# videosegmentation/video_segment

Hardware: AMD Instinct MI355X
Metric: over-segmented frames/sec at 1080p (higher is better)
Workload: dtype f32

## Files before the change

### video_segment_amd/csrc/dense_graph.cpp

```cpp
#include "dense_graph.h"
#include "scan_device.h"

#include <algorithm>
#include <chrono>
#include <cmath>
#include <cstring>
#include <atomic>
#include <functional>
#include <thread>
#include <unordered_set>

namespace vsg {

namespace {
template <class T>
DevBuf<T>& Grow(DevBuf<T>& b, size_t n) {
  if (b.size() < n) b.alloc(n + n / 2 + 1024);
  return b;
}
double NowMs() {
  using clk = std::chrono::steady_clock;
  return std::chrono::duration<double, std::milli>(clk::now().time_since_epoch()).count();
}
template <class T>
// ... 577 lines not shown
  const int window_bushy = getenv("VSG_WINDOW_BUSHY") ? atoi(getenv("VSG_WINDOW_BUSHY")) : 64;
  const bool adapt_windows = !getenv("VSG_ADAPT_WINDOWS") || atoi(getenv("VSG_ADAPT_WINDOWS")) != 0;
  const int window_min_edges =
      getenv("VSG_WINDOW_MIN") ? atoi(getenv("VSG_WINDOW_MIN")) : (int)std::min<size_t>(2 * wh_, 1u << 30);
  const int window_min_replayed =
      getenv("VSG_WINDOW_MIN_REPLAYED") ? atoi(getenv("VSG_WINDOW_MIN_REPLAYED"))
                                        : (getenv("VSG_WINDOW_MIN") ? 0 : (int)std::min<size_t>(wh_ / 2, 1u << 30));
  S.bucket_prefix = bucket_prefix_dev_.get();
  S.bucket_prefix_host = bucket_prefix.data();
  {
    list_off_host_.assign((size_t)L * (kNumBuckets + 2), 0);
    for (int l = 0; l < L; ++l) {
      int32_t* off = list_off_host_.data() + (size_t)l * (kNumBuckets + 2);
      int acc_l = 0;
      for (int b = 0; b <= kNumBuckets; ++b) {
        off[b] = acc_l;
        const int32_t* row = bucket_base_host_.data() + (size_t)b * (L + 1);
        acc_l += row[l + 1] - row[l];
      }
      off[kNumBuckets + 1] = acc_l;
    }
    const size_t cap = (size_t)3 * 65536;
    if (seg_table_dev_.size() < cap) seg_table_dev_.alloc(cap);
    S.bucket_base_host = getenv("VSG_FILTER_SEGS") && atoi(getenv("VSG_FILTER_SEGS")) == 0 ? nullptr
                                                                                          : bucket_base_host_.data();
    S.list_off_host = list_off_host_.data();
    S.list_slot_base_host = list_slot_base_.data();
    S.seg_dev = seg_table_dev_.get();
    S.seg_cap = seg_table_dev_.size();
    S.seg_host = &seg_table_host_;
  }
  if (++window_target_age_ > 8) {
    window_target_age_ = 0;
    for (size_t b = 0; b < window_target_.size(); ++b) {
      int64_t& t = window_target_[b];
      if (t != 0 && t != kNoWindowTarget && window_peak_[b] <= 4096) t = t * 2 > (1ll << 28) ? 0 : t * 2;
    }
    std::fill(window_peak_.begin(), window_peak_.end(), 0);
    std::fill(window_last_seg_.begin(), window_last_seg_.end(), 0);
    std::fill(window_frozen_.begin(), window_frozen_.end(), 0);
    std::fill(window_unpaid_.begin(), window_unpaid_.end(), 0);
  }
  int group_width = 1;
  double low_bucket_ms[2] = {0, 0};
  for (int b = 0, hi = 0; b < kNumBuckets; b = hi) {
    const double t_bucket0 = b < 2 ? NowMs() : 0;
    struct LowBucketTimer {
      double* out;
      double t0;
      ~LowBucketTimer() { if (out) *out += NowMs() - t0; }
    } low_timer{b < 2 ? &low_bucket_ms[b] : nullptr, t_bucket0};
    hi = b + 1;
    if (group_buckets && b >= first_plain) {
// ... 1117 lines not shown
```

### video_segment_amd/csrc/dense_graph.h

```cpp
#ifndef VSG_DENSE_GRAPH_H_
#define VSG_DENSE_GRAPH_H_

#include <memory>
#include <unordered_map>
#include <vector>

#include "device_graph.h"
#include "host_model.h"

namespace vsg {

struct MergePaths {
  int64_t hub_stages = 0, hub_absorbed = 0;
  int64_t hub_cuts = 0, hub_cuts_in_groups = 0, hub_parts_in_later_bucket = 0, spine_side_cuts = 0;
  int64_t hub_retries = 0, hub_reasons[6] = {0, 0, 0, 0, 0, 0};
  int64_t hub_exclusion_reruns = 0, hub_off_reruns = 0, group_halvings = 0, conservative_replays = 0;
};

struct GraphTimings {
  float edges_ms = 0, sort_ms = 0, merge_ms = 0, readout_ms = 0, host_post_ms = 0;
  int64_t edges_total = 0, edges_active = 0;
  int64_t merges[3] = {0, 0, 0};
  float wave_ms = 0, filter_ms = 0, spine_ms = 0;
  int64_t wave_launches = 0, filter_launches = 0, wave_edges = 0, spine_launches = 0, spine_edges = 0;
// ... 108 lines not shown
  std::vector<int32_t> bucket_base_host_;
  DevBuf<uint16_t> keys_tmp_;
  DevBuf<int32_t> hist_tmp_, hist_sums_;
  DevBuf<int32_t> first_label_scratch_;
  DevBuf<int32_t> e_ra_, e_rb_;
  DevBuf<uint32_t> e_gpos_;
  DevBuf<uint8_t> active_slab_;
  struct ActiveArrays {
    int32_t *e_active = nullptr, *e_apos = nullptr, *a_ra = nullptr, *a_rb = nullptr, *seg_cnt = nullptr,
            *seg_off = nullptr, *lead_pos = nullptr, *l_ra = nullptr, *l_rb = nullptr, *bk_cons = nullptr;
    uint32_t *a_gpos = nullptr, *a_comp = nullptr, *a_idx = nullptr, *s_comp = nullptr, *s_idx = nullptr,
             *seg_key = nullptr, *l_gpos = nullptr;
    float4* bk_ds = nullptr;
    uint8_t* bk_flags = nullptr;
  } act_;
  DevBuf<unsigned long long> filter_masks_;
  DevBuf<int32_t> block_cnt_, block_off_;
  int64_t optimistic_stages_ = 0, rollbacks_ = 0;
  DevBuf<int32_t> scalars_;
  DevBuf<int32_t> seg_table_dev_;
  DevBuf<int32_t> hub_excl_;
  PinnedBuf<int32_t> iv_host_;
  std::vector<int32_t> seg_table_host_, list_off_host_;
  Mailbox mail_;
  void* mail_mem_ = nullptr;
  DevBuf<int32_t> zero_pool_mem_;
  ZeroPool zero_pool_;
  DevBuf<int32_t> bucket_prefix_dev_;
  int spine_limit_bucket_ = 0x7fffffff;
  int spine_limit_age_ = 0;
  int spine_low_fails_[2] = {0, 0}, spine_low_cooldown_[2] = {0, 0};
  double spine_low_cost_fail_[2] = {0, 0}, spine_low_cost_skip_[2] = {0, 0};
  int spine_low_cost_age_[2] = {0, 0};
  DevBuf<int32_t> spine_pool_;
  static constexpr int64_t kNoWindowTarget = 1ll << 40;
  int64_t wave_target_active_ = kNoWindowTarget;
  std::vector<int64_t> window_target_;
  int window_target_age_ = 0;
  std::vector<int> window_last_seg_;
  std::vector<uint8_t> window_frozen_;
  std::vector<uint8_t> window_unpaid_;
  std::vector<int> window_peak_;
  std::vector<int> hub_bucket_stages_, hub_bucket_pause_;
  std::vector<long long> hub_bucket_absorbed_;
  double last_density_ = 1.0;
  int spine_max_edges_grown_ = 0;
// ... 35 lines not shown
```

### video_segment_amd/csrc/device_graph.h

```cpp
#ifndef VSG_DEVICE_GRAPH_H_
#define VSG_DEVICE_GRAPH_H_

#include <functional>

#include "common.h"

namespace vsg {

constexpr uint8_t kFlagFinalized = 1;
constexpr uint8_t kFlagNoDesc = 2;
constexpr uint8_t kFlagTentative = 4;
constexpr uint8_t kFlagHub = 8;
constexpr uint8_t kFlagHubBroken = 16;
constexpr uint8_t kFlagHubExcluded = 32;
constexpr int kHubExclCap = 16384;
constexpr int kHubMaxAttempts = 4;
constexpr int kHubMaxSplits = 64;
constexpr int kHubCutCap = 64;
constexpr int kHubListInts = 4 + kHubExclCap + 3 * kHubCutCap;

struct NodeArrays {
  int32_t* parent;
  float4* desc_sz;
  int32_t* cons;
// ... 97 lines not shown
struct MailWaitCounters {
  long long waits = 0;
  double wait_ms = 0, longest_ms = 0;
};
MailWaitCounters MailWaitSnapshot();
void MailWaitResetLongest();
void LaunchMailPost(const MailSlot& slot, const int32_t* p0, const int32_t* p1, const int32_t* p2,
                    const int32_t* p3, hipStream_t s);

constexpr size_t kZeroArenaInts = 1024;
struct ZeroPool {
  int32_t* base = nullptr;
  size_t cap = 0, used = 0;
  bool second_half = false;
  size_t arena_used = 0;
};

struct FilterMasks {
  unsigned long long* active;
  unsigned long long* settled;
  unsigned long long* tentative;
  int32_t* block_cnt;
};
struct FilterSegs {
  const int32_t* start;
  const int32_t* list;
  const int32_t* pos0;
  int n;
};
struct MergeScratch {
  int active_cap;
  std::function<bool(long long need)> grow_active;
  int32_t* e_ra;
  int32_t* e_rb;
  uint32_t* e_gpos;
  int32_t* e_active;
  int32_t* e_apos;
  FilterMasks masks;
  int32_t* block_off;
  int32_t* a_ra;
  int32_t* a_rb;
  uint32_t* a_gpos;
  uint32_t* a_comp;
  uint32_t* a_idx;
  uint32_t* s_comp;
  uint32_t* s_idx;
  uint32_t* seg_key;
  int32_t* seg_cnt;
  int32_t* seg_off;
  int32_t* num_active;
  int32_t* num_segs;
  float4* bk_ds;
  int32_t* bk_cons;
  uint8_t* bk_flags;
  int force_rollback;
  int32_t* lead_pos;
  int32_t* l_ra;
  int32_t* l_rb;
  uint32_t* l_gpos;
  int use_rle;
  int group_hi;
  const int32_t* bucket_prefix;
  const int32_t* bucket_prefix_host;
  const int32_t* bucket_base_host;
  const int32_t* list_off_host;
  int32_t* seg_dev;
  size_t seg_cap;
  std::vector<int32_t>* seg_host;
  int spine_min;
  int spine_off;
  int* spine_low_failed;
  const int* spine_low_skip;
  int* spine_limit_bucket;
  int spine_nested_factor;
  int spine_max_edges;
  int spine_debug, spine_check;
  int rank_split_min;
  int spine_fast;
  int spine_fast_min;
  int32_t* spine_pool;
  size_t spine_pool_ints;
  std::function<bool(long long edges)> grow_spine_pool;
  int32_t* nmap[3];
  hipStream_t aux_stream;
  hipStream_t aux2_stream;
  hipEvent_t aux_fork, aux_join;
  int small_seg;
  int wide_min;
  int wide_waves;
  int chain_relax;
  int hubs;
// ... 21 lines not shown
  int wave_debug;
  int wave_dbg;
  int64_t* optimistic_stages;
  int64_t* rollbacks;
  int32_t* cc;
  unsigned long long* stats;
  void* cub_temp;
  size_t cub_temp_bytes;
  ScanScratch scan;
  int node_key_bits;
  std::vector<hipEvent_t>* ev_pool;
  std::vector<std::pair<int, int>>* ev_wave;
  std::vector<std::pair<int, int>>* ev_filter;
  std::vector<std::pair<int, int>>* ev_spine;
  int* ev_used;
  Mailbox* mail;
  ZeroPool* zeros;
  hipStream_t main_stream;
};
int32_t* TakeZeroed(MergeScratch& S, size_t n);

int32_t* TakeStageScalars(MergeScratch& S, size_t n);

void LaunchBuildBucketTable(const ListDesc* lists, int num_lists, int32_t* bucket_base,
                            hipStream_t s);
void LaunchInitIdentity(int32_t* a, size_t n, hipStream_t s);
struct StageInfo {
  int want_components = 0;
  int replayed = 0;
  int components = 0;
  int max_wave_segment = 0;
  int hub_stages = 0;
  long long hub_absorbed = 0;
  int hub_retries = 0;
};
void ResetHubExclusions(MergeScratch& S, NodeArrays nodes, hipStream_t s);
void RunBucketStage(int bucket, int j0, int n_b, const ListDesc* lists, const int32_t* bucket_base,
                    const uint32_t* list_slot_base, uint8_t* kept_all, NodeArrays nodes,
                    const MergeParams& P, int inert_mode, MergeScratch& S, hipStream_t s,
                    StageInfo* info = nullptr);
size_t SpinePoolInts(size_t max_edges);
void LaunchKeepVirtualBucket(const ListDesc* lists, int num_lists, hipStream_t s);

void LaunchFlatten(NodeArrays nodes, size_t n, int32_t* label_uf, hipStream_t s);
void LaunchEnforceN4(int32_t* label_img, int W, int H, const int32_t* frames_dev, int num_frames,
                     int32_t* row_flags , int32_t* adjust ,
// ... 53 lines not shown
```

### video_segment_amd/csrc/merge_spine.hip

```cpp
#include <algorithm>
#include <chrono>
#include <cstdlib>
#include <cstdio>
#include <unordered_map>
#include <vector>

#include "merge_common.h"
#include "scan_device.h"

namespace vsg {

namespace {

constexpr int kNone = -1;

static inline unsigned Blocks(size_t n) { return (unsigned)((n + 255) / 256); }

__device__ __forceinline__ int CompOf(const int32_t* __restrict__ comp_base, int K, int e) {
  int lo = 0, hi = K;
  while (hi - lo > 1) {
    const int mid = (lo + hi) >> 1;
    if (comp_base[mid] <= e) lo = mid; else hi = mid;
  }
  return lo;
// ... 1218 lines not shown
  };
  Mark(0);
  if (pool_used >= S.spine_pool_ints) return false;
  Pool pool{S.spine_pool + pool_used, S.spine_pool_ints - pool_used};
  int32_t* d_base = pool.take(K + 1);
  int32_t* d_off = pool.take(K);
  int32_t* root_vertex = pool.take(K);
  int32_t* comp_spine = pool.take(K + 1);
  unsigned long long* root_key = reinterpret_cast<unsigned long long*>(TakeZeroed(S, 2 * (size_t)K));
  int32_t* scalars = pool.take(64);
  int32_t* eu = pool.take(mE);
  int32_t* ev = pool.take(mE);
  int32_t* estate = pool.take(mE);
  int32_t* flag = pool.take(mE);
  int32_t* scan = pool.take(mE);
  int32_t* side_key = pool.take(mE);
  int32_t* spine_flag = pool.take(mE);
  if (!pool.ok) return false;
  int32_t* cc = S.cc;
  uint32_t* best = reinterpret_cast<uint32_t*>(S.nmap[0]);
  int32_t* firstq = S.nmap[1];
  int32_t* childidx = S.nmap[2];

  VSG_HIP(hipMemcpyAsync(d_base, base.data(), (K + 1) * sizeof(int32_t), hipMemcpyHostToDevice, s));
  VSG_HIP(hipMemcpyAsync(d_off, off.data(), K * sizeof(int32_t), hipMemcpyHostToDevice, s));
  hipLaunchKernelGGL(k_spine_gather, dim3(Blocks(mE)), dim3(256), 0, s, mE, K, d_base, d_off, wa.s_ra,
                     wa.s_rb, eu, ev, estate, cc, best);
  hipLaunchKernelGGL(k_spine_pick_root, dim3(Blocks((size_t)K + (mE + kRootStride - 1) / kRootStride)), dim3(256), 0,
                     s, mE, K, eu, ev, d_base, wa.nodes, root_key);
  hipLaunchKernelGGL(k_spine_roots, dim3((K + 63) / 64), dim3(64), 0, s, K, root_key, root_vertex, childidx);

  int dbg_rounds = 0;
  auto NowMs = [] {
    return std::chrono::duration<double, std::milli>(std::chrono::steady_clock::now().time_since_epoch()).count();
  };
  const bool dbg_big = S.spine_debug && mE > (8 << 20);
  if (dbg_big) {
    VSG_HIP(hipStreamSynchronize(s));
    std::fprintf(stderr, "[vsg]   forest: gather+root %.2f ms\n", NowMs() - tph[0]);
  }
  {
    const size_t forest_mark = pool.mark();
    const int32_t* list = nullptr;
    const int32_t* list_len = nullptr;
    int n_list = mE;
    int32_t* lists[2] = {nullptr, nullptr};
    int which = 0;
    const int ahead_max = getenv("VSG_BOR_AHEAD") ? atoi(getenv("VSG_BOR_AHEAD")) : (4 << 20);
// ... 320 lines not shown
```

### video_segment_amd/csrc/merge_stage.hip

```cpp
#include <sched.h>
#include <time.h>

#include <algorithm>
#include <atomic>
#include <chrono>
#include <thread>
#include <vector>

#include "merge_common.h"
#include "scan_device.h"

namespace vsg {

__global__ __launch_bounds__(256) void k_build_bucket_table(const ListDesc* __restrict__ lists,
                                                             int num_lists,
                                                             int32_t* __restrict__ bucket_base) {
  const int b = blockIdx.x * 256 + threadIdx.x;
  if (b > kNumBuckets) return;
  int acc = 0;
  int32_t* row = bucket_base + (size_t)b * (num_lists + 1);
  for (int l = 0; l < num_lists; ++l) {
    row[l] = acc;
    const int32_t* off = lists[l].offsets;
    if (off) acc += off[b + 1] - off[b];
  }
  row[num_lists] = acc;
}

void LaunchBuildBucketTable(const ListDesc* lists, int num_lists, int32_t* bucket_base,
// ... 120 lines not shown
    z.used = 0;
    VSG_HIP(hipMemsetAsync(z.base + kZeroArenaInts + (z.second_half ? half : 0), 0, half * sizeof(int32_t),
                           S.main_stream));
  }
  int32_t* p = z.base + kZeroArenaInts + (z.second_half ? half : 0) + z.used;
  z.used += n;
  return p;
}

int32_t* TakeStageScalars(MergeScratch& S, size_t n) {
  ZeroPool& z = *S.zeros;
  n = (n + 3) & ~(size_t)3;
  VSG_REQUIRE(n <= kZeroArenaInts, -4, "zero pool: stage scalars too large");
  if (z.arena_used + n > kZeroArenaInts) {
    DrainStreams(S);
    VSG_HIP(hipMemsetAsync(z.base, 0, kZeroArenaInts * sizeof(int32_t), S.main_stream));
    z.arena_used = 0;
  }
  int32_t* p = z.base + z.arena_used;
  z.arena_used += n;
  return p;
}

constexpr int kFilterPer = 2;
constexpr int kFilterEdges = 256 * kFilterPer;

__global__ __launch_bounds__(256) void k_filter(int bucket, int bucket_hi, int j0, int n_b,
                                                 const ListDesc* __restrict__ lists,
                                                 const int32_t* __restrict__ bucket_base,
                                                 const int32_t* __restrict__ bucket_prefix,
                                                 const uint32_t* __restrict__ list_slot_base,
                                                 uint8_t* __restrict__ kept_all, NodeArrays nodes,
                                                 MergeParams P, int inert_mode,
                                                 int32_t* __restrict__ cc,
                                                 int32_t* __restrict__ e_ra,
                                                 int32_t* __restrict__ e_rb,
                                                 uint32_t* __restrict__ e_gpos,
                                                 FilterMasks M,
                                                 int32_t* __restrict__ num_ti, FilterSegs segs, int hubs,
                                                 int32_t* __restrict__ num_hub, int32_t* __restrict__ hub_excl,
                                                 float split_s) {
  __shared__ int wave_cnt[kFilterPer][4], wave_kept[kFilterPer][4];
  __shared__ int s_start[kFilterEdges], s_pos0[kFilterEdges];
  __shared__ const uint32_t* s_slots[kFilterEdges];
  __shared__ const int32_t* s_prev[kFilterEdges];
  __shared__ int s_type[kFilterEdges], s_base_a[kFilterEdges], s_base_b[kFilterEdges];
  __shared__ uint32_t s_slot_base[kFilterEdges];
  const int jf = blockIdx.x * kFilterEdges;
  int m_segs = 0;
  if (segs.start) {
    int first = 0;
    if (segs.n > kFilterEdges) {
      const int stride = (segs.n + 255) / 256;
      const int t1 = threadIdx.x * stride;
      const int c1 = __syncthreads_count(t1 < segs.n && segs.start[t1] <= jf);
      const int base = (c1 - 1) * stride;
      const int t2 = base + threadIdx.x;
      const int c2 = __syncthreads_count(threadIdx.x < stride && t2 < segs.n && segs.start[t2] <= jf);
      first = base + c2 - 1;
    }
    m_segs = min(kFilterEdges, segs.n - first);
    for (int i = threadIdx.x; i < m_segs; i += 256) {
      s_start[i] = segs.start[first + i];
      const int l = segs.list[first + i];
      s_pos0[i] = segs.pos0[first + i];
      const ListDesc L = lists[l];
      s_slots[i] = L.slots;
      s_prev[i] = L.type != 0 ? L.prev_idx : reinterpret_cast<const int32_t*>(L.slots);
      s_type[i] = L.type;
      s_base_a[i] = L.base_a;
      s_base_b[i] = L.base_b;
      s_slot_base[i] = list_slot_base[l];
    }
    __syncthreads();
  }
  bool valid[kFilterPer];
  int a[kFilterPer], b[kFilterPer], l_type[kFilterPer];
  uint32_t gpos[kFilterPer];
  if (segs.start) {
    const uint32_t* slots_p[kFilterPer];
    const int32_t* prev_p[kFilterPer];
    int pos[kFilterPer], base_a[kFilterPer], base_b[kFilterPer];
#pragma unroll
    for (int e = 0; e < kFilterPer; ++e) {
      const int j = jf + e * 256 + threadIdx.x;
      valid[e] = j < n_b;
      const int jc = valid[e] ? j : n_b - 1;
      int lo = 0, hi = m_segs;
      while (hi - lo > 1) {
        const int mid = (lo + hi) >> 1;
        if (s_start[mid] <= jc) lo = mid; else hi = mid;
      }
      pos[e] = s_pos0[lo] + (jc - s_start[lo]);
      slots_p[e] = s_slots[lo];
      prev_p[e] = s_prev[lo];
      l_type[e] = s_type[lo];
      base_a[e] = s_base_a[lo];
      base_b[e] = s_base_b[lo];
      gpos[e] = s_slot_base[lo] + (uint32_t)pos[e];
    }
    uint32_t slot[kFilterPer];
#pragma unroll
    for (int e = 0; e < kFilterPer; ++e) slot[e] = slots_p[e][pos[e]];
    uint32_t pix[kFilterPer];
    int pv[kFilterPer];
#pragma unroll
    for (int e = 0; e < kFilterPer; ++e) {
      const uint32_t tm = (uint32_t)-(int)(l_type[e] != 0);
      pix[e] = ((slot[e] / 9u) & tm) | ((slot[e] >> 2) & ~tm);
      pv[e] = prev_p[e][pix[e]];
    }
#pragma unroll
    for (int e = 0; e < kFilterPer; ++e) {
      a[e] = base_a[e] + (int)pix[e];
      const int kt = (int)(slot[e] - pix[e] * 9u);
      const int dy = kt / 3 - 1, dx = kt - (kt / 3) * 3 - 1;
      const int bt = base_b[e] + pv[e] + dy * P.W + dx;
      const int ks = (int)(slot[e] & 3u);
      const int bs = a[e] + (ks != 0 ? P.W : 0) + (ks == 0 || ks == 3 ? 1 : 0) - (ks == 2 ? 1 : 0);
      const int tm = -(int)(l_type[e] != 0);
      b[e] = (bt & tm) | (bs & ~tm);
    }
// ... 11 lines not shown
        while (hi - lo > 1) {
          const int mid = (lo + hi) >> 1;
          if (bucket_prefix[mid] <= jg) lo = mid; else hi = mid;
        }
        bk = lo;
        jb = jg - bucket_prefix[bk];
      }
      const int32_t* base_row = bucket_base + (size_t)bk * (P.num_lists + 1);
      const int l = LocateList(base_row, P.num_lists, jb);
      const int pos = lists[l].offsets[bk] + (jb - base_row[l]);
      const ListDesc L = lists[l];
      l_type[e] = L.type;
      DecodeEdge(L, L.slots[pos], P.W, a[e], b[e]);
      gpos[e] = list_slot_base[l] + (uint32_t)pos;
    }
  }
  constexpr int kChains = 2 * kFilterPer;
  int x0[kChains], root[kChains];
#pragma unroll
  for (int e = 0; e < kFilterPer; ++e) {
    x0[2 * e] = a[e];
    x0[2 * e + 1] = b[e];
  }
#pragma unroll
  for (int c = 0; c < kChains; ++c) root[c] = x0[c];
  for (bool any = true; any;) {
    int p[kChains];
#pragma unroll
    for (int c = 0; c < kChains; ++c) p[c] = nodes.parent[root[c]];
    any = false;
#pragma unroll
    for (int c = 0; c < kChains; ++c) {
      if (p[c] != root[c]) {
        root[c] = p[c];
        any = true;
      }
    }
  }
  {
    int cur[kChains];
#pragma unroll
    for (int c = 0; c < kChains; ++c) cur[c] = x0[c];
    for (bool any = true; any;) {
      int nx[kChains];
#pragma unroll
      for (int c = 0; c < kChains; ++c) nx[c] = cur[c] != root[c] ? nodes.parent[cur[c]] : root[c];
      any = false;
#pragma unroll
      for (int c = 0; c < kChains; ++c) {
        if (cur[c] != root[c]) {
          if (nx[c] != root[c]) nodes.parent[cur[c]] = root[c];
          cur[c] = nx[c];
          any = any || (cur[c] != root[c]);
        }
      }
    }
  }
  int ti[kFilterPer], active[kFilterPer], settled[kFilterPer];
#pragma unroll
  for (int e = 0; e < kFilterPer; ++e) {
    ti[e] = active[e] = settled[e] = 0;
    const int ra = root[2 * e], rb = root[2 * e + 1];
    if (!valid[e] || ra == rb) continue;
    if (P.spatial_survivors && l_type[e] == 0 && !P.spatial_survivors[gpos[e]]) continue;
    bool inert = false;
    int f1 = 0, f2 = 0, s1 = 0, s2 = 0, c1 = -1, c2 = -1;
// ... 204 lines not shown
  if (blockIdx.x == gridDim.x - 1 && threadIdx.x == 255) {
    const int total = base + (int)__popcll(m);
    *num_active = total;
    MailPost(mail, mail_seq, 0, total);
    MailPost(mail, mail_seq, 1, *num_ti);
    MailPost(mail, mail_seq, 2, *num_hub);
  }
}

__global__ __launch_bounds__(256) void k_component_ids(int n, const int32_t* __restrict__ a_ra,
                                                        int32_t* __restrict__ cc,
                                                        uint32_t* __restrict__ a_comp,
                                                        uint32_t* __restrict__ a_idx) {
  const int i = blockIdx.x * 256 + threadIdx.x;
  if (i >= n) return;
  a_comp[i] = (uint32_t)CcFind(cc, a_ra[i]);
  a_idx[i] = (uint32_t)i;
}

__global__ __launch_bounds__(256) void k_reset_cc(int n, const int32_t* __restrict__ a_ra,
                                                   const int32_t* __restrict__ a_rb,
                                                   int32_t* __restrict__ cc,
                                                   const int32_t* __restrict__ violation,
                                                   unsigned long long* __restrict__ mail, unsigned mail_seq) {
  const int i = blockIdx.x * 256 + threadIdx.x;
  if (i == 0 && mail) MailPost(mail, mail_seq, 0, *violation);
  if (i >= n) return;
  const int ra = a_ra[i], rb = a_rb[i];
  cc[ra] = ra;
  cc[rb] = rb;
}

__global__ __launch_bounds__(256) void k_gather_sorted(int n, const uint32_t* __restrict__ s_idx,
                                                        const int32_t* __restrict__ a_ra,
                                                        const int32_t* __restrict__ a_rb,
                                                        const uint32_t* __restrict__ a_gpos,
                                                        int32_t* __restrict__ s_ra,
                                                        int32_t* __restrict__ s_rb,
                                                        uint32_t* __restrict__ s_gpos) {
  const int p = blockIdx.x * 256 + threadIdx.x;
  if (p >= n) return;
  const uint32_t i = s_idx[p];
  s_ra[p] = a_ra[i];
  s_rb[p] = a_rb[i];
  s_gpos[p] = a_gpos[i];
}


__global__ __launch_bounds__(256) void k_merge_small(const int32_t* __restrict__ num_segs,
                                                      const int32_t* __restrict__ seg_off,
                                                      const int32_t* __restrict__ seg_cnt,
                                                      const int32_t* __restrict__ s_ra,
                                                      const int32_t* __restrict__ s_rb,
                                                      const uint32_t* __restrict__ s_gpos,
                                                      NodeArrays nodes, uint8_t* __restrict__ kept_all,
                                                      StageThr T, int optimistic,
                                                      int32_t* __restrict__ violation,
                                                      unsigned long long* __restrict__ stats,
                                                      int small_seg, int wave_max,
                                                      uint32_t* __restrict__ work_list,
                                                      int work_cap, int32_t* __restrict__ work_ctl,
                                                      int cls_min0, int32_t* __restrict__ hub_mark,
                                                      const uint32_t* __restrict__ s_seq,
                                                      int32_t* __restrict__ hub_excl) {
  const int seg = blockIdx.x * 256 + threadIdx.x;
  unsigned n_forced = 0, n_regular = 0, n_small = 0;
  const int cnt = seg < *num_segs ? seg_cnt[seg] : 0;
  if (work_list) {
// ... 446 lines not shown
  const bool try_hubs = S.hubs && !S.hubs_off && inert_mode != 0 && !spine_possible && S.wide_min <= 0;
  if (S.hub_excl && S.hub_list_dirty) {
    if (S.hub_attempt == 0) {
      VSG_HIP(hipMemsetAsync(S.hub_excl, 0, 4 * sizeof(int32_t), s));
      S.hub_list_dirty = 0;
    } else {
      VSG_HIP(hipMemsetAsync(S.hub_excl + 1, 0, 3 * sizeof(int32_t), s));
    }
  }
  if (S.hub_excl && S.hub_check) {
    int head[4] = {0, 0, 0, 0};
    VSG_HIP(hipMemcpyAsync(head, S.hub_excl, sizeof(head), hipMemcpyDeviceToHost, s));
    VSG_HIP(hipStreamSynchronize(s));
    for (int k = 1; k < 4; ++k) {
      if (head[k] != 0) {
        Throw(-4 , "hub check: stage b=" + std::to_string(bucket) + " j0=" + std::to_string(j0) +
                                             " n=" + std::to_string(n_b) + " starts with " + std::to_string(head[k]) +
                                             " stale entries of kind " + std::to_string(k - 1) + " on the hub list");
      }
    }
  }
  if (S.hub_attempt == 0 && S.hub_split_depth == 0) S.hub_splits_left = S.hub_max_splits;
  int32_t* d_num_leaders = S.num_active + 5;
  FilterSegs segs = {nullptr, nullptr, nullptr, 0};
  if (S.bucket_base_host && S.list_off_host && S.seg_dev) {
    const int L = P.num_lists;
    std::vector<int32_t>& h = *S.seg_host;
    h.clear();
    const int64_t g0 = (int64_t)S.bucket_prefix_host[bucket] + j0, g1 = g0 + n_b;
    std::vector<int32_t> st, li, po;
    for (int b = bucket; b < bucket_hi; ++b) {
      const int32_t* row = S.bucket_base_host + (size_t)b * (L + 1);
      const int64_t bstart = S.bucket_prefix_host[b];
      if (bstart + row[L] <= g0) continue;
      if (bstart >= g1) break;
      for (int l = 0; l < L; ++l) {
        const int cnt = row[l + 1] - row[l];
        if (cnt == 0) continue;
        const int64_t s0 = bstart + row[l], s1 = s0 + cnt;
        if (s1 <= g0 || s0 >= g1) continue;
        const int64_t first = std::max(s0, g0);
        st.push_back((int32_t)(first - g0));
        li.push_back(l);
        po.push_back(S.list_off_host[(size_t)l * (kNumBuckets + 2) + b] + (int32_t)(first - s0));
      }
    }
    const int nseg = (int)st.size();
    if (nseg > 0 && nseg <= 65536 && (size_t)3 * nseg <= S.seg_cap) {
      h.reserve((size_t)3 * nseg);
      h.insert(h.end(), st.begin(), st.end());
      h.insert(h.end(), li.begin(), li.end());
      h.insert(h.end(), po.begin(), po.end());
      VSG_HIP(hipMemcpyAsync(S.seg_dev, h.data(), h.size() * sizeof(int32_t), hipMemcpyHostToDevice, s));
      segs.start = S.seg_dev;
      segs.list = S.seg_dev + nseg;
      segs.pos0 = S.seg_dev + 2 * (size_t)nseg;
      segs.n = nseg;
    }
  }
  const float split_s = ((float)bucket * P.inv_scale < P.force_merge_weight) ? P.s_lt_02 : P.s_le_015;
  const int ef0 = NextEvent(S);
  if (ef0 >= 0) VSG_HIP(hipEventRecord((*S.ev_pool)[ef0], s));
  hipLaunchKernelGGL(k_filter, dim3((unsigned)((n_b + kFilterEdges - 1) / kFilterEdges)), dim3(256), 0, s, bucket, bucket_hi, j0, n_b, lists,
                     bucket_base, S.bucket_prefix, list_slot_base, kept_all, nodes, P, inert_mode, S.cc, S.e_ra, S.e_rb, S.e_gpos,
                     S.masks, d_num_ti, segs, try_hubs ? 1 : 0, d_num_hub, S.hub_excl, split_s);
  const int ef1 = NextEvent(S);
  if (ef1 >= 0) {
    VSG_HIP(hipEventRecord((*S.ev_pool)[ef1], s));
    S.ev_filter->emplace_back(ef0, ef1);
  }
  if (try_hubs) hipLaunchKernelGGL(k_hub_check, dim3(16), dim3(256), 0, s, S.hub_excl, nodes, d_num_hub);
  ExclusiveSum(S.scan, S.masks.block_cnt, S.block_off, (int)Blocks(n_b), s);
  int h[3] = {0, 0, 0};
  for (int attempt = 0;; ++attempt) {
    const MailSlot m_active = NextMail(*S.mail);
    hipLaunchKernelGGL(k_compact_active, dim3(Blocks(n_b)), dim3(256), 0, s, n_b, S.masks, S.block_off,
                       S.e_ra, S.e_rb, S.e_gpos, S.a_ra, S.a_rb, S.a_gpos, S.num_active, d_num_ti, m_active.dev,
                       m_active.seq, S.active_cap, d_num_hub);
    VSG_HIP(hipGetLastError());
    MailWait(m_active, 3, h, s);
    if (h[0] <= S.active_cap) break;
    VSG_REQUIRE(attempt == 0 && S.grow_active && S.grow_active(h[0]) && h[0] <= S.active_cap, -4,
                "stage scratch: cannot hold the active edges");
  }
  const int n_active = h[0];
  const int n_ti = h[1];
  const bool hubs_used = try_hubs && (h[2] & 1) != 0;
  if (h[2] & (8 | 16)) S.hub_list_dirty = 1;
// ... 142 lines not shown
        ++replayed;
        prev = c + 1;
      }
      part(prev, n_b - prev, false);
      if (info) info->replayed = replayed;
      return true;
    }
    if (violated & (kVioCut | 2)) return false;
    int& depth = (list_complete && S.hub_attempt + 1 < kHubMaxAttempts) ? S.hub_attempt : S.hubs_off;
    if (&depth == &S.hub_attempt) {
      hipLaunchKernelGGL(k_hub_exclude, dim3(16), dim3(256), 0, s, S.hub_excl, nodes);
      ++S.hub_exclusion_reruns;
    } else {
      ++S.hub_off_reruns;
    }
    ++depth;
    RunBucketStage(bucket, j0, n_b, lists, bucket_base, list_slot_base, kept_all, nodes, P, inert_mode, S, s, info);
    --depth;
    if (S.hub_attempt == 0 && S.hubs_off == 0) ResetHubExclusions(S, nodes, s);
    return true;
  };
  if (hubs_used && ((h[2] & 6) != 0 || ((h[2] & 16) != 0 && can_cut(n_active, (long long)(h[2] >> 8))))) {
    hipLaunchKernelGGL(k_reset_cc, dim3(Blocks(n_active)), dim3(256), 0, s, n_active, S.a_ra, S.a_rb, S.cc,
                       d_violation, nullptr, 0u);
    hipLaunchKernelGGL(k_clear_kept, dim3(Blocks(n_b)), dim3(256), 0, s, n_b, S.masks, S.e_gpos, kept_all);
    clear_marks();
    clear_hub_marks();
    VSG_HIP(hipGetLastError());
    if (retry_without_broken_hubs(kHubVioBroken, n_active, (h[2] & 4) == 0, nullptr)) return;
    VSG_REQUIRE(false, -4, "hub stage: no way to rerun it");
  }
  if (hubs_used && info) ++info->hub_stages;

  const bool rle = S.use_rle && inert_mode != 0 && n_active >= 64;
  const int32_t* w_ra = S.a_ra;
  const int32_t* w_rb = S.a_rb;
  const uint32_t* w_gpos = S.a_gpos;
  int n_work = n_active;
  int32_t* lead = S.e_active;
  if (rle) {
    const MailSlot m_lead = NextMail(*S.mail);
    FusedScan(S.scan, LeaderValue{S.a_ra, S.a_rb},
              LeaderEmit{S.a_ra, S.a_rb, S.a_gpos, lead, S.lead_pos, S.l_ra, S.l_rb, S.l_gpos},
              LeaderFinish{d_num_leaders, m_lead.dev, m_lead.seq}, n_active, s);
    MailWait(m_lead, 1, &n_work, s);
    w_ra = S.l_ra;
    w_rb = S.l_rb;
// ... 18 lines not shown
    }
  }
  const bool spine = !spine_in.segs.empty();
  VSG_REQUIRE(!(spine && hubs_used), -4, "merge stage: hub regions in a stage with a tree replay");
  const bool optimistic = ((inert_mode == 2) && (n_ti > 0 || rle)) || spine || hubs_used;
  if (optimistic) {
    hipLaunchKernelGGL(k_backup_roots, dim3(Blocks(n_work)), dim3(256), 0, s, n_work, w_ra, w_rb,
                       nodes, S.bk_ds, S.bk_cons, S.bk_flags, S.stats);
  }

  const float weight = (float)bucket * P.inv_scale;
  const bool force = weight < P.force_merge_weight;
  StageThr T;
  T.pass_s = force ? P.s_lt_02 : P.s_lt_005;
  T.split_s = force ? P.s_lt_02 : P.s_le_015;
  T.min_size = P.min_region_size;
  T.rle = rle ? 1 : 0;
  T.side = 0;
  T.relax = S.chain_relax;
  T.hubs = hubs_used ? 1 : 0;
  int32_t* s_ra = reinterpret_cast<int32_t*>(S.a_comp);
  int32_t* s_rb = reinterpret_cast<int32_t*>(S.a_idx);
  uint32_t* s_gpos = reinterpret_cast<uint32_t*>(S.e_apos);
  hipLaunchKernelGGL(k_gather_sorted, dim3(Blocks(n_work)), dim3(256), 0, s, n_work, S.s_idx, w_ra,
                     w_rb, w_gpos, s_ra, s_rb, s_gpos);
  const int small_seg = S.small_seg;
  auto WaveGrid = [small_seg](int n) {
    const int g = n / (small_seg + 1);
    return g < 1 ? 1 : (g > 8192 ? 8192 : g);
  };
  const int wave_grid = WaveGrid(n_work);
  WorkerArgs wa;
  wa.num_segs = S.num_segs;
  wa.seg_off = S.seg_off;
  wa.seg_cnt = S.seg_cnt;
  wa.s_ra = s_ra;
  wa.s_rb = s_rb;
  wa.s_gpos = s_gpos;
  wa.nodes = nodes;
  wa.kept_all = kept_all;
  wa.T = T;
  wa.optimistic = optimistic ? 1 : 0;
  wa.violation = d_violation;
  wa.stats = S.stats;
  wa.small_seg = small_seg;
  wa.wave_min = small_seg;
  wa.wave_max = spine_thr;
  wa.work_cap = n_work / (small_seg + 1) + 1;
// ... 64 lines not shown
    int32_t* run_off = reinterpret_cast<int32_t*>(S.seg_key);
    int32_t* run_cnt = S.seg_off;
    const MailSlot m_hub = NextMail(*S.mail);
    FusedScan(S.scan, HubMarkValue{wa.hub_mark}, HubMarkEmit{wa.hub_mark, nodes.parent, seq_list, key_list},
              HubMarkFinish{d_hub_count, m_hub.dev, m_hub.seq}, n_work, s);
    int n_abs = 0;
    MailWait(m_hub, 1, &n_abs, s);
    if (n_abs > 0) {
      SortPairsU32(S.cub_temp, S.cub_temp_bytes, key_list, key_sorted, seq_list, seq_sorted, n_abs, S.node_key_bits, s);
      RunsOfSortedKeys(S.scan, key_sorted, n_abs, run_off, run_cnt, d_hub_runs, s);
      hipLaunchKernelGGL(k_hub_apply, dim3((unsigned)((n_abs + 63) / 64)), dim3(64), 0, s, d_hub_runs, run_off,
                         run_cnt, key_sorted, seq_sorted, wa.hub_mark, nodes, T.split_s, d_violation, S.hub_excl);
      if (n_abs >= kHubWaveMin) {
        hipLaunchKernelGGL(k_hub_apply_wave, dim3((unsigned)std::min(n_abs / kHubWaveMin, 2048)), dim3(64), 0, s,
                           d_hub_runs, run_off, run_cnt, key_sorted, seq_sorted, wa.hub_mark, nodes, T.split_s,
                           d_violation, S.hub_excl);
      }
    }
    if (info) info->hub_absorbed += n_abs;
  }
  MailSlot m_vio = {nullptr, nullptr, 0};
  if (optimistic) m_vio = NextMail(*S.mail);
  hipLaunchKernelGGL(k_reset_cc, dim3(Blocks(n_work)), dim3(256), 0, s, n_work, w_ra, w_rb, S.cc, d_violation,
                     m_vio.dev, m_vio.seq);
  VSG_HIP(hipGetLastError());
  if (optimistic) {
    int violated = 0;
    MailWait(m_vio, 1, &violated, s);
    ++*S.optimistic_stages;
    if (violated || S.force_rollback) {
      ++*S.rollbacks;
      S.hub_list_dirty = 1;
      hipLaunchKernelGGL(k_restore_roots, dim3(Blocks(n_work)), dim3(256), 0, s, n_work, w_ra, w_rb,
                         nodes, S.bk_ds, S.bk_cons, S.bk_flags, S.stats);
      hipLaunchKernelGGL(k_clear_kept, dim3(Blocks(n_b)), dim3(256), 0, s, n_b, S.masks, S.e_gpos, kept_all);
      clear_marks();
      clear_hub_marks();
      VSG_HIP(hipGetLastError());
      if (spine && violated == 2 && bucket < 2 && !S.force_rollback && retry_without_broken_hubs(2, n_work, true, w_gpos)) {
        return;
      }
      if (spine && violated == 2 && !S.force_rollback) {
        if (bucket >= 2 && bucket < *S.spine_limit_bucket) *S.spine_limit_bucket = bucket;
        if (bucket < 2) S.spine_low_failed[bucket] = 1;
        const int off = S.spine_off;
        S.spine_off = 1;
        RunBucketStage(bucket, j0, n_b, lists, bucket_base, list_slot_base, kept_all, nodes, P, inert_mode, S,
                       s, info);
        S.spine_off = off;
        return;
      }
// ... 10 lines not shown
        int replayed = 0;
        for (const auto& h : halves) {
          const int64_t lo = std::max<int64_t>(g0, S.bucket_prefix_host[h[0]]);
          const int64_t hi = std::min<int64_t>(g1, S.bucket_prefix_host[h[1]]);
          if (hi <= lo) continue;
          S.group_hi = h[1];
          StageInfo sub;
          RunBucketStage(h[0], (int)(lo - S.bucket_prefix_host[h[0]]), (int)(hi - lo), lists, bucket_base,
                         list_slot_base, kept_all, nodes, P, inert_mode, S, s, info ? &sub : nullptr);
          replayed += sub.replayed;
        }
        S.group_hi = group_hi;
        if (info) info->replayed = replayed;
        return;
      }
      ++S.conservative_replays;
      RunBucketStage(bucket, j0, n_b, lists, bucket_base, list_slot_base, kept_all, nodes, P, 0, S,
                     s, info);
      return;
    }
  }
  if (info) {
    info->replayed = n_work;
    if (info->want_components && (info->want_components > 1 || n_work > 16384)) {
      int32_t* d_max = TakeZeroed(S, 1);
      hipLaunchKernelGGL(k_max_segment, dim3(Blocks(n_work)), dim3(256), 0, s, n_work, S.num_segs, S.seg_cnt,
                         spine ? spine_thr : 0x7fffffff, d_max);
      const MailSlot m_info = NextMail(*S.mail);
      LaunchMailPost(m_info, S.num_segs, d_max, nullptr, nullptr, s);
      int v[2] = {0, 0};
      MailWait(m_info, 2, v, s);
      info->components = v[0];
      info->max_wave_segment = v[1];
    }
  }
  if (rle && n_work < n_active) {
    hipLaunchKernelGGL(k_resolve_followers, dim3(Blocks(n_active)), dim3(256), 0, s, n_active, lead,
                       S.lead_pos, S.a_gpos, S.l_gpos, kept_all);
  }
  clear_marks();
  clear_hub_marks();
  VSG_HIP(hipGetLastError());
}

__global__ __launch_bounds__(256) void k_run_counts(int n, const int32_t* __restrict__ num_runs,
                                                     const int32_t* __restrict__ seg_off,
                                                     int32_t* __restrict__ seg_cnt) {
// ... 45 lines not shown
```

Before: 204.2.

## Pass filter segments as kernel args, batch host uploads, fold stats into mail

```diff
diff --git a/video_segment_amd/csrc/dense_graph.cpp b/video_segment_amd/csrc/dense_graph.cpp
--- a/video_segment_amd/csrc/dense_graph.cpp
+++ b/video_segment_amd/csrc/dense_graph.cpp
@@ -623,13 +623,18 @@
     }
     const size_t cap = (size_t)3 * 65536;
     if (seg_table_dev_.size() < cap) seg_table_dev_.alloc(cap);
-    S.bucket_base_host = getenv("VSG_FILTER_SEGS") && atoi(getenv("VSG_FILTER_SEGS")) == 0 ? nullptr
-                                                                                          : bucket_base_host_.data();
+    S.filter_segs_mode = getenv("VSG_FILTER_SEGS") ? atoi(getenv("VSG_FILTER_SEGS")) : 2;
+    S.bucket_base_host = S.filter_segs_mode == 0 ? nullptr : bucket_base_host_.data();
+    S.lists_host = desc.data();
     S.list_off_host = list_off_host_.data();
     S.list_slot_base_host = list_slot_base_.data();
     S.seg_dev = seg_table_dev_.get();
     S.seg_cap = seg_table_dev_.size();
     S.seg_host = &seg_table_host_;
+    stage_ring_.ensure(kStageRingInts);
+    S.ring_host = stage_ring_.get();
+    S.ring_cap = stage_ring_.size();
+    S.ring_used = &stage_ring_used_;
   }
   if (++window_target_age_ > 8) {
     window_target_age_ = 0;
diff --git a/video_segment_amd/csrc/dense_graph.h b/video_segment_amd/csrc/dense_graph.h
--- a/video_segment_amd/csrc/dense_graph.h
+++ b/video_segment_amd/csrc/dense_graph.h
@@ -154,6 +154,8 @@
   DevBuf<int32_t> hub_excl_;
   PinnedBuf<int32_t> iv_host_;
   std::vector<int32_t> seg_table_host_, list_off_host_;
+  size_t stage_ring_used_ = 0;
+  PinnedBuf<int32_t> stage_ring_;
   Mailbox mail_;
   void* mail_mem_ = nullptr;
   DevBuf<int32_t> zero_pool_mem_;
diff --git a/video_segment_amd/csrc/device_graph.h b/video_segment_amd/csrc/device_graph.h
--- a/video_segment_amd/csrc/device_graph.h
+++ b/video_segment_amd/csrc/device_graph.h
@@ -143,12 +143,21 @@
   unsigned long long* tentative;
   int32_t* block_cnt;
 };
+struct FilterSegRec {
+  const uint32_t* slots;
+  const int32_t* prev;
+  int32_t start, pos0, type, base_a, base_b;
+  uint32_t slot_base;
+};
+constexpr int kFilterArgSegs = 64;
+struct FilterSegArgs {
+  FilterSegRec r[kFilterArgSegs];
+};
 struct FilterSegs {
-  const int32_t* start;
-  const int32_t* list;
-  const int32_t* pos0;
+  const FilterSegRec* rec;
   int n;
 };
+constexpr size_t kStageRingInts = (size_t)1 << 18;
 struct MergeScratch {
   int active_cap;
   std::function<bool(long long need)> grow_active;
@@ -188,6 +197,10 @@
   int32_t* seg_dev;
   size_t seg_cap;
   std::vector<int32_t>* seg_host;
+  const ListDesc* lists_host;
+  int filter_segs_mode;
+  int32_t* ring_host;
+  size_t ring_cap, *ring_used;
   int spine_min;
   int spine_off;
   int* spine_low_failed;
@@ -255,6 +268,8 @@
 
 int32_t* TakeStageScalars(MergeScratch& S, size_t n);
 
+int32_t* TakeStageRing(MergeScratch& S, size_t n);
+
 void LaunchBuildBucketTable(const ListDesc* lists, int num_lists, int32_t* bucket_base,
                             hipStream_t s);
 void LaunchInitIdentity(int32_t* a, size_t n, hipStream_t s);
diff --git a/video_segment_amd/csrc/merge_spine.hip b/video_segment_amd/csrc/merge_spine.hip
--- a/video_segment_amd/csrc/merge_spine.hip
+++ b/video_segment_amd/csrc/merge_spine.hip
@@ -1264,8 +1264,17 @@
   int32_t* firstq = S.nmap[1];
   int32_t* childidx = S.nmap[2];
 
-  VSG_HIP(hipMemcpyAsync(d_base, base.data(), (K + 1) * sizeof(int32_t), hipMemcpyHostToDevice, s));
-  VSG_HIP(hipMemcpyAsync(d_off, off.data(), K * sizeof(int32_t), hipMemcpyHostToDevice, s));
+  VSG_REQUIRE(d_off == d_base + (((size_t)K + 1 + 63) & ~(size_t)63), -4, "spine: off does not follow base in the pool");
+  const size_t off_at = (size_t)(d_off - d_base);
+  if (int32_t* src = TakeStageRing(S, off_at + K)) {
+    std::copy(base.begin(), base.end(), src);
+    std::fill(src + K + 1, src + off_at, 0);
+    std::copy(off.begin(), off.end(), src + off_at);
+    VSG_HIP(hipMemcpyAsync(d_base, src, (off_at + K) * sizeof(int32_t), hipMemcpyHostToDevice, s));
+  } else {
+    VSG_HIP(hipMemcpyAsync(d_base, base.data(), (K + 1) * sizeof(int32_t), hipMemcpyHostToDevice, s));
+    VSG_HIP(hipMemcpyAsync(d_off, off.data(), K * sizeof(int32_t), hipMemcpyHostToDevice, s));
+  }
   hipLaunchKernelGGL(k_spine_gather, dim3(Blocks(mE)), dim3(256), 0, s, mE, K, d_base, d_off, wa.s_ra,
                      wa.s_rb, eu, ev, estate, cc, best);
   hipLaunchKernelGGL(k_spine_pick_root, dim3(Blocks((size_t)K + (mE + kRootStride - 1) / kRootStride)), dim3(256), 0,
diff --git a/video_segment_amd/csrc/merge_stage.hip b/video_segment_amd/csrc/merge_stage.hip
--- a/video_segment_amd/csrc/merge_stage.hip
+++ b/video_segment_amd/csrc/merge_stage.hip
@@ -4,7 +4,9 @@
 #include <algorithm>
 #include <atomic>
 #include <chrono>
+#include <cstring>
 #include <thread>
+#include <type_traits>
 #include <vector>
 
 #include "merge_common.h"
@@ -171,9 +173,22 @@
   return p;
 }
 
+int32_t* TakeStageRing(MergeScratch& S, size_t n) {
+  n = (n + 15) & ~(size_t)15;
+  if (!S.ring_host || n > S.ring_cap) return nullptr;
+  if (*S.ring_used + n > S.ring_cap) {
+    DrainStreams(S);
+    *S.ring_used = 0;
+  }
+  int32_t* p = S.ring_host + *S.ring_used;
+  *S.ring_used += n;
+  return p;
+}
+
 constexpr int kFilterPer = 2;
 constexpr int kFilterEdges = 256 * kFilterPer;
 
+template <bool kArgs>
 __global__ __launch_bounds__(256) void k_filter(int bucket, int bucket_hi, int j0, int n_b,
                                                  const ListDesc* __restrict__ lists,
                                                  const int32_t* __restrict__ bucket_base,
@@ -186,67 +201,97 @@
                                                  int32_t* __restrict__ e_rb,
                                                  uint32_t* __restrict__ e_gpos,
                                                  FilterMasks M,
-                                                 int32_t* __restrict__ num_ti, FilterSegs segs, int hubs,
+                                                 int32_t* __restrict__ num_ti, FilterSegs segs,
+                                                 std::conditional_t<kArgs, FilterSegArgs, int> A, int hubs,
                                                  int32_t* __restrict__ num_hub, int32_t* __restrict__ hub_excl,
                                                  float split_s) {
+  constexpr int kSegCap = kArgs ? 1 : kFilterEdges;
   __shared__ int wave_cnt[kFilterPer][4], wave_kept[kFilterPer][4];
-  __shared__ int s_start[kFilterEdges], s_pos0[kFilterEdges];
-  __shared__ const uint32_t* s_slots[kFilterEdges];
-  __shared__ const int32_t* s_prev[kFilterEdges];
-  __shared__ int s_type[kFilterEdges], s_base_a[kFilterEdges], s_base_b[kFilterEdges];
-  __shared__ uint32_t s_slot_base[kFilterEdges];
+  __shared__ int s_start[kSegCap], s_pos0[kSegCap];
+  __shared__ const uint32_t* s_slots[kSegCap];
+  __shared__ const int32_t* s_prev[kSegCap];
+  __shared__ int s_type[kSegCap], s_base_a[kSegCap], s_base_b[kSegCap];
+  __shared__ uint32_t s_slot_base[kSegCap];
   const int jf = blockIdx.x * kFilterEdges;
+  const bool have_segs = kArgs || segs.rec != nullptr;
   int m_segs = 0;
-  if (segs.start) {
-    int first = 0;
-    if (segs.n > kFilterEdges) {
-      const int stride = (segs.n + 255) / 256;
-      const int t1 = threadIdx.x * stride;
-      const int c1 = __syncthreads_count(t1 < segs.n && segs.start[t1] <= jf);
-      const int base = (c1 - 1) * stride;
-      const int t2 = base + threadIdx.x;
-      const int c2 = __syncthreads_count(threadIdx.x < stride && t2 < segs.n && segs.start[t2] <= jf);
-      first = base + c2 - 1;
-    }
-    m_segs = min(kFilterEdges, segs.n - first);
-    for (int i = threadIdx.x; i < m_segs; i += 256) {
-      s_start[i] = segs.start[first + i];
-      const int l = segs.list[first + i];
-      s_pos0[i] = segs.pos0[first + i];
-      const ListDesc L = lists[l];
-      s_slots[i] = L.slots;
-      s_prev[i] = L.type != 0 ? L.prev_idx : reinterpret_cast<const int32_t*>(L.slots);
-      s_type[i] = L.type;
-      s_base_a[i] = L.base_a;
-      s_base_b[i] = L.base_b;
-      s_slot_base[i] = list_slot_base[l];
-    }
-    __syncthreads();
+  if constexpr (!kArgs) {
+    if (segs.rec) {
+      int first = 0;
+      if (segs.n > kFilterEdges) {
+        const int stride = (segs.n + 255) / 256;
+        const int t1 = threadIdx.x * stride;
+        const int c1 = __syncthreads_count(t1 < segs.n && segs.rec[t1].start <= jf);
+        const int base = (c1 - 1) * stride;
+        const int t2 = base + threadIdx.x;
+        const int c2 = __syncthreads_count(threadIdx.x < stride && t2 < segs.n && segs.rec[t2].start <= jf);
+        first = base + c2 - 1;
+      }
+      m_segs = min(kFilterEdges, segs.n - first);
+      for (int i = threadIdx.x; i < m_segs; i += 256) {
+        const FilterSegRec R = segs.rec[first + i];
+        s_start[i] = R.start;
+        s_pos0[i] = R.pos0;
+        s_slots[i] = R.slots;
+        s_prev[i] = R.prev;
+        s_type[i] = R.type;
+        s_base_a[i] = R.base_a;
+        s_base_b[i] = R.base_b;
+        s_slot_base[i] = R.slot_base;
+      }
+      __syncthreads();
+    }
   }
   bool valid[kFilterPer];
   int a[kFilterPer], b[kFilterPer], l_type[kFilterPer];
   uint32_t gpos[kFilterPer];
-  if (segs.start) {
+  if (have_segs) {
     const uint32_t* slots_p[kFilterPer];
     const int32_t* prev_p[kFilterPer];
     int pos[kFilterPer], base_a[kFilterPer], base_b[kFilterPer];
+    int jc[kFilterPer];
 #pragma unroll
     for (int e = 0; e < kFilterPer; ++e) {
       const int j = jf + e * 256 + threadIdx.x;
       valid[e] = j < n_b;
-      const int jc = valid[e] ? j : n_b - 1;
-      int lo = 0, hi = m_segs;
-      while (hi - lo > 1) {
-        const int mid = (lo + hi) >> 1;
-        if (s_start[mid] <= jc) lo = mid; else hi = mid;
-      }
-      pos[e] = s_pos0[lo] + (jc - s_start[lo]);
-      slots_p[e] = s_slots[lo];
-      prev_p[e] = s_prev[lo];
-      l_type[e] = s_type[lo];
-      base_a[e] = s_base_a[lo];
-      base_b[e] = s_base_b[lo];
-      gpos[e] = s_slot_base[lo] + (uint32_t)pos[e];
+      jc[e] = valid[e] ? j : n_b - 1;
+    }
+    if constexpr (kArgs) {
+      const int lane = threadIdx.x & 63;
+      const int st = lane < segs.n ? A.r[lane].start : 0x7fffffff;
+      const int first = max(0, (int)__popcll(__ballot(st <= jf)) - 1);
+      const int end = max(first + 1, (int)__popcll(__ballot(st < min(jf + kFilterEdges, n_b))));
+      for (int k = first; k < end; ++k) {
+        const FilterSegRec R = A.r[k];
+#pragma unroll
+        for (int e = 0; e < kFilterPer; ++e) {
+          if (k == first || jc[e] >= R.start) {
+            pos[e] = R.pos0 + (jc[e] - R.start);
+            slots_p[e] = R.slots;
+            prev_p[e] = R.prev;
+            l_type[e] = R.type;
+            base_a[e] = R.base_a;
+            base_b[e] = R.base_b;
+            gpos[e] = R.slot_base + (uint32_t)pos[e];
+          }
+        }
+      }
+    } else {
+#pragma unroll
+      for (int e = 0; e < kFilterPer; ++e) {
+        int lo = 0, hi = m_segs;
+        while (hi - lo > 1) {
+          const int mid = (lo + hi) >> 1;
+          if (s_start[mid] <= jc[e]) lo = mid; else hi = mid;
+        }
+        pos[e] = s_pos0[lo] + (jc[e] - s_start[lo]);
+        slots_p[e] = s_slots[lo];
+        prev_p[e] = s_prev[lo];
+        l_type[e] = s_type[lo];
+        base_a[e] = s_base_a[lo];
+        base_b[e] = s_base_b[lo];
+        gpos[e] = s_slot_base[lo] + (uint32_t)pos[e];
+      }
     }
     uint32_t slot[kFilterPer];
 #pragma unroll
@@ -304,9 +349,16 @@
     x0[2 * e] = a[e];
     x0[2 * e + 1] = b[e];
   }
-#pragma unroll
-  for (int c = 0; c < kChains; ++c) root[c] = x0[c];
-  for (bool any = true; any;) {
+  int hop[kChains];
+#pragma unroll
+  for (int c = 0; c < kChains; ++c) hop[c] = nodes.parent[x0[c]];
+  bool any = false;
+#pragma unroll
+  for (int c = 0; c < kChains; ++c) {
+    root[c] = hop[c];
+    any = any || (hop[c] != x0[c]);
+  }
+  while (any) {
     int p[kChains];
 #pragma unroll
     for (int c = 0; c < kChains; ++c) p[c] = nodes.parent[root[c]];
@@ -322,8 +374,15 @@
   {
     int cur[kChains];
 #pragma unroll
-    for (int c = 0; c < kChains; ++c) cur[c] = x0[c];
-    for (bool any = true; any;) {
+    for (int c = 0; c < kChains; ++c) {
+      cur[c] = root[c];
+      if (x0[c] != root[c] && hop[c] != root[c]) {
+        nodes.parent[x0[c]] = root[c];
+        cur[c] = hop[c];
+        any = true;
+      }
+    }
+    while (any) {
       int nx[kChains];
 #pragma unroll
       for (int c = 0; c < kChains; ++c) nx[c] = cur[c] != root[c] ? nodes.parent[cur[c]] : root[c];
@@ -574,9 +633,16 @@
                                                    const int32_t* __restrict__ a_rb,
                                                    int32_t* __restrict__ cc,
                                                    const int32_t* __restrict__ violation,
-                                                   unsigned long long* __restrict__ mail, unsigned mail_seq) {
+                                                   unsigned long long* __restrict__ mail, unsigned mail_seq,
+                                                   const int32_t* __restrict__ decomp) {
   const int i = blockIdx.x * 256 + threadIdx.x;
-  if (i == 0 && mail) MailPost(mail, mail_seq, 0, *violation);
+  if (i == 0 && mail) {
+    MailPost(mail, mail_seq, 0, *violation);
+    if (decomp) {
+      MailPost(mail, mail_seq, 1, decomp[1]);
+      MailPost(mail, mail_seq, 2, decomp[0]);
+    }
+  }
   if (i >= n) return;
   const int ra = a_ra[i], rb = a_rb[i];
   cc[ra] = ra;
@@ -589,13 +655,25 @@
                                                         const uint32_t* __restrict__ a_gpos,
                                                         int32_t* __restrict__ s_ra,
                                                         int32_t* __restrict__ s_rb,
-                                                        uint32_t* __restrict__ s_gpos) {
+                                                        uint32_t* __restrict__ s_gpos,
+                                                        const int32_t* __restrict__ num_segs,
+                                                        const int32_t* __restrict__ seg_cnt, int below,
+                                                        int32_t* __restrict__ decomp) {
   const int p = blockIdx.x * 256 + threadIdx.x;
-  if (p >= n) return;
-  const uint32_t i = s_idx[p];
-  s_ra[p] = a_ra[i];
-  s_rb[p] = a_rb[i];
-  s_gpos[p] = a_gpos[i];
+  if (p < n) {
+    const uint32_t i = s_idx[p];
+    s_ra[p] = a_ra[i];
+    s_rb[p] = a_rb[i];
+    s_gpos[p] = a_gpos[i];
+  }
+  if (decomp) {
+    const int m = *num_segs;
+    int v = p < n && p < m ? seg_cnt[p] : 0;
+    if (v >= below) v = 0;
+    for (int off = 32; off > 0; off >>= 1) v = max(v, __shfl_xor(v, off));
+    if ((threadIdx.x & 63) == 0 && v > decomp[0]) atomicMax(decomp, v);
+    if (p == 0) decomp[1] = m;
+  }
 }
 
 
@@ -1088,13 +1166,14 @@
   }
   if (S.hub_attempt == 0 && S.hub_split_depth == 0) S.hub_splits_left = S.hub_max_splits;
   int32_t* d_num_leaders = S.num_active + 5;
-  FilterSegs segs = {nullptr, nullptr, nullptr, 0};
-  if (S.bucket_base_host && S.list_off_host && S.seg_dev) {
+  FilterSegs segs = {nullptr, 0};
+  FilterSegArgs seg_args;
+  bool segs_in_args = false;
+  if (S.bucket_base_host && S.list_off_host && S.lists_host && S.list_slot_base_host && S.seg_dev) {
     const int L = P.num_lists;
-    std::vector<int32_t>& h = *S.seg_host;
-    h.clear();
+    constexpr size_t kRecInts = sizeof(FilterSegRec) / sizeof(int32_t);
     const int64_t g0 = (int64_t)S.bucket_prefix_host[bucket] + j0, g1 = g0 + n_b;
-    std::vector<int32_t> st, li, po;
+    std::vector<FilterSegRec> recs;
     for (int b = bucket; b < bucket_hi; ++b) {
       const int32_t* row = S.bucket_base_host + (size_t)b * (L + 1);
       const int64_t bstart = S.bucket_prefix_host[b];
@@ -1106,30 +1185,49 @@
         const int64_t s0 = bstart + row[l], s1 = s0 + cnt;
         if (s1 <= g0 || s0 >= g1) continue;
         const int64_t first = std::max(s0, g0);
-        st.push_back((int32_t)(first - g0));
-        li.push_back(l);
-        po.push_back(S.list_off_host[(size_t)l * (kNumBuckets + 2) + b] + (int32_t)(first - s0));
-      }
-    }
-    const int nseg = (int)st.size();
-    if (nseg > 0 && nseg <= 65536 && (size_t)3 * nseg <= S.seg_cap) {
-      h.reserve((size_t)3 * nseg);
-      h.insert(h.end(), st.begin(), st.end());
-      h.insert(h.end(), li.begin(), li.end());
-      h.insert(h.end(), po.begin(), po.end());
-      VSG_HIP(hipMemcpyAsync(S.seg_dev, h.data(), h.size() * sizeof(int32_t), hipMemcpyHostToDevice, s));
-      segs.start = S.seg_dev;
-      segs.list = S.seg_dev + nseg;
-      segs.pos0 = S.seg_dev + 2 * (size_t)nseg;
+        const ListDesc& D = S.lists_host[l];
+        FilterSegRec R;
+        R.slots = D.slots;
+        R.prev = D.type != 0 ? D.prev_idx : reinterpret_cast<const int32_t*>(D.slots);
+        R.start = (int32_t)(first - g0);
+        R.pos0 = S.list_off_host[(size_t)l * (kNumBuckets + 2) + b] + (int32_t)(first - s0);
+        R.type = D.type;
+        R.base_a = D.base_a;
+        R.base_b = D.base_b;
+        R.slot_base = S.list_slot_base_host[l];
+        recs.push_back(R);
+      }
+    }
+    const int nseg = (int)recs.size();
+    if (nseg > 0 && nseg <= kFilterArgSegs && S.filter_segs_mode != 1) {
+      std::copy(recs.begin(), recs.end(), seg_args.r);
+      segs.n = nseg;
+      segs_in_args = true;
+    } else if (nseg > 0 && nseg <= 65536 && kRecInts * nseg <= S.seg_cap) {
+      int32_t* src = TakeStageRing(S, kRecInts * nseg);
+      if (!src) {
+        S.seg_host->resize(kRecInts * nseg);
+        src = S.seg_host->data();
+      }
+      std::memcpy(src, recs.data(), (size_t)nseg * sizeof(FilterSegRec));
+      VSG_HIP(hipMemcpyAsync(S.seg_dev, src, (size_t)nseg * sizeof(FilterSegRec), hipMemcpyHostToDevice, s));
+      segs.rec = reinterpret_cast<const FilterSegRec*>(S.seg_dev);
       segs.n = nseg;
     }
   }
   const float split_s = ((float)bucket * P.inv_scale < P.force_merge_weight) ? P.s_lt_02 : P.s_le_015;
   const int ef0 = NextEvent(S);
   if (ef0 >= 0) VSG_HIP(hipEventRecord((*S.ev_pool)[ef0], s));
-  hipLaunchKernelGGL(k_filter, dim3((unsigned)((n_b + kFilterEdges - 1) / kFilterEdges)), dim3(256), 0, s, bucket, bucket_hi, j0, n_b, lists,
-                     bucket_base, S.bucket_prefix, list_slot_base, kept_all, nodes, P, inert_mode, S.cc, S.e_ra, S.e_rb, S.e_gpos,
-                     S.masks, d_num_ti, segs, try_hubs ? 1 : 0, d_num_hub, S.hub_excl, split_s);
+  const dim3 filter_grid((unsigned)((n_b + kFilterEdges - 1) / kFilterEdges));
+  if (segs_in_args) {
+    hipLaunchKernelGGL(k_filter<true>, filter_grid, dim3(256), 0, s, bucket, bucket_hi, j0, n_b, lists, bucket_base,
+                       S.bucket_prefix, list_slot_base, kept_all, nodes, P, inert_mode, S.cc, S.e_ra, S.e_rb, S.e_gpos,
+                       S.masks, d_num_ti, segs, seg_args, try_hubs ? 1 : 0, d_num_hub, S.hub_excl, split_s);
+  } else {
+    hipLaunchKernelGGL(k_filter<false>, filter_grid, dim3(256), 0, s, bucket, bucket_hi, j0, n_b, lists, bucket_base,
+                       S.bucket_prefix, list_slot_base, kept_all, nodes, P, inert_mode, S.cc, S.e_ra, S.e_rb, S.e_gpos,
+                       S.masks, d_num_ti, segs, 0, try_hubs ? 1 : 0, d_num_hub, S.hub_excl, split_s);
+  }
   const int ef1 = NextEvent(S);
   if (ef1 >= 0) {
     VSG_HIP(hipEventRecord((*S.ev_pool)[ef1], s));
@@ -1318,7 +1416,7 @@
   };
   if (hubs_used && ((h[2] & 6) != 0 || ((h[2] & 16) != 0 && can_cut(n_active, (long long)(h[2] >> 8))))) {
     hipLaunchKernelGGL(k_reset_cc, dim3(Blocks(n_active)), dim3(256), 0, s, n_active, S.a_ra, S.a_rb, S.cc,
-                       d_violation, nullptr, 0u);
+                       d_violation, nullptr, 0u, nullptr);
     hipLaunchKernelGGL(k_clear_kept, dim3(Blocks(n_b)), dim3(256), 0, s, n_b, S.masks, S.e_gpos, kept_all);
     clear_marks();
     clear_hub_marks();
@@ -1383,8 +1481,10 @@
   int32_t* s_ra = reinterpret_cast<int32_t*>(S.a_comp);
   int32_t* s_rb = reinterpret_cast<int32_t*>(S.a_idx);
   uint32_t* s_gpos = reinterpret_cast<uint32_t*>(S.e_apos);
+  const bool report = info && info->want_components && (info->want_components > 1 || n_work > 16384);
+  int32_t* d_decomp = report && optimistic ? d_num_ti + 5 : nullptr;
   hipLaunchKernelGGL(k_gather_sorted, dim3(Blocks(n_work)), dim3(256), 0, s, n_work, S.s_idx, w_ra,
-                     w_rb, w_gpos, s_ra, s_rb, s_gpos);
+                     w_rb, w_gpos, s_ra, s_rb, s_gpos, S.num_segs, S.seg_cnt, spine ? spine_thr : 0x7fffffff, d_decomp);
   const int small_seg = S.small_seg;
   auto WaveGrid = [small_seg](int n) {
     const int g = n / (small_seg + 1);
@@ -1495,11 +1595,15 @@
   MailSlot m_vio = {nullptr, nullptr, 0};
   if (optimistic) m_vio = NextMail(*S.mail);
   hipLaunchKernelGGL(k_reset_cc, dim3(Blocks(n_work)), dim3(256), 0, s, n_work, w_ra, w_rb, S.cc, d_violation,
-                     m_vio.dev, m_vio.seq);
+                     m_vio.dev, m_vio.seq, d_decomp);
   VSG_HIP(hipGetLastError());
+  int decomp[2] = {0, 0};
   if (optimistic) {
-    int violated = 0;
-    MailWait(m_vio, 1, &violated, s);
+    int vio[3] = {0, 0, 0};
+    MailWait(m_vio, d_decomp ? 3 : 1, vio, s);
+    const int violated = vio[0];
+    decomp[0] = vio[1];
+    decomp[1] = vio[2];
     ++*S.optimistic_stages;
     if (violated || S.force_rollback) {
       ++*S.rollbacks;
@@ -1556,7 +1660,10 @@
   }
   if (info) {
     info->replayed = n_work;
-    if (info->want_components && (info->want_components > 1 || n_work > 16384)) {
+    if (d_decomp) {
+      info->components = decomp[0];
+      info->max_wave_segment = decomp[1];
+    } else if (report) {
       int32_t* d_max = TakeZeroed(S, 1);
       hipLaunchKernelGGL(k_max_segment, dim3(Blocks(n_work)), dim3(256), 0, s, n_work, S.num_segs, S.seg_cnt,
                          spine ? spine_thr : 0x7fffffff, d_max);
```

New measurement: 207.8 (median of 6 runs). 1.8% higher.
